# hrnr/map-merge

Measured on AMD Instinct MI355X. Metric: map-pairs/sec (normals+FPFH+SAC-IA+ICP, end to end incl. per-map features), higher is better.
Workload: dtype f32; 1 GPU; 16 maps x 500000 raw pts, FPFH + SAC_IA + ICP refine, 120 pairs; parallelism=one mm3d_estimate_maps_transforms call, 16 streams inside the library, points_after_filter_mean=406681, keypoints_mean=15692

## Files before the change

include/mm3d.h:

```cpp
#ifndef MM3D_H_
#define MM3D_H_

#include <stddef.h>
#include <stdint.h>

#ifdef __cplusplus
extern "C" {
#endif

typedef enum {
  MM3D_OK = 0,
  MM3D_EINVAL = -1,
  MM3D_EDEVICE = -2,
  MM3D_ENOMEM = -3,
  MM3D_EUNSUPPORTED = -4,
  MM3D_ECAPACITY = -5
} mm3d_status;

typedef enum { MM3D_DESC_PFH = 0, MM3D_DESC_PFHRGB, MM3D_DESC_FPFH, MM3D_DESC_RSD, MM3D_DESC_SHOT, MM3D_DESC_SC3D } mm3d_descriptor;
typedef enum { MM3D_KP_SIFT = 0, MM3D_KP_HARRIS } mm3d_keypoint;
typedef enum { MM3D_EST_MATCHING = 0, MM3D_EST_SAC_IA } mm3d_estimation_method;
typedef enum { MM3D_ICP_POINT_TO_POINT = 0, MM3D_ICP_POINT_TO_PLANE = 1 } mm3d_icp_method;

const char *mm3d_descriptor_name(int d);
// ... 26 lines not shown
void mm3d_params_default(mm3d_params *p);
int mm3d_params_from_command_line(int argc, const char *const *argv, mm3d_params *p);
size_t mm3d_params_to_string(const mm3d_params *p, char *buf, size_t cap);

typedef struct { int32_t index_query, index_match; float distance; } mm3d_corr;

typedef struct mm3d_ctx mm3d_ctx;
typedef struct mm3d_cloud mm3d_cloud;
typedef struct mm3d_normals mm3d_normals;
typedef struct mm3d_desc mm3d_desc;

int mm3d_create(int device, mm3d_ctx **out);
int mm3d_create_devices(const int *devices, int n_devices, mm3d_ctx **out);
int mm3d_device_count(const mm3d_ctx *ctx);
int mm3d_device_at(const mm3d_ctx *ctx, int i);
int mm3d_devices_use_rccl(const mm3d_ctx *ctx);
void mm3d_destroy(mm3d_ctx *ctx);
const char *mm3d_last_error(const mm3d_ctx *ctx);
int mm3d_last_icp_iterations(const mm3d_ctx *ctx);
int mm3d_last_icp_converged(const mm3d_ctx *ctx);
void mm3d_set_debug(mm3d_ctx *ctx, int on);
long long mm3d_debug_knn_fallback_rows(mm3d_ctx *ctx);
long long mm3d_debug_knn_rows(mm3d_ctx *ctx);
void mm3d_debug_waits(mm3d_ctx *ctx, long long out[2]);
int mm3d_debug_float_chain(mm3d_ctx *ctx, const float *incr, const unsigned *hits, int n, float *out);
int mm3d_debug_libm(mm3d_ctx *ctx, int fn, const float *x, const float *y, int n, float *out);
int mm3d_debug_pair_bins(mm3d_ctx *ctx, const float *p1, const float *n1, const float *p2, const float *n2, int n, int *out);
int mm3d_debug_sacia_queries_per_thread(int k);
int mm3d_debug_wave_primitives(mm3d_ctx *ctx, int op, const void *in, int n, void *out_new, void *out_old);
int mm3d_debug_sift_cert_octave(mm3d_ctx *ctx, const mm3d_cloud *points, double min_scale, int octave, float *val, float *bound,
                                size_t capacity, size_t *n_out);
void mm3d_debug_sift_cert_stats(long long out[8], int reset);
void mm3d_debug_sift_cert_min(int n);
float mm3d_debug_cloud_voxel_leaf(const mm3d_cloud *cloud);
void mm3d_debug_sacia_stats(long long out[4], int reset, int collect);
int mm3d_debug_desc_knn(mm3d_ctx *ctx, const float *a, size_t na, const float *b, size_t nb, int dim, int k, int *idx, float *d2);
typedef struct mm3d_nn_search_info {
  float max_d2;
  float rmax;
  float cell;
  float origin[3];
  int dims[3];
  int max_ring;
  int n_items;
} mm3d_nn_search_info;
int mm3d_debug_nn_search(mm3d_ctx *ctx, const mm3d_cloud *source, const mm3d_cloud *target, const float T[16], double range,
                         int convention, int split, int *idx, float *d2, mm3d_nn_search_info *info);
void mm3d_srand(mm3d_ctx *ctx, unsigned seed);
int mm3d_set_streams(mm3d_ctx *ctx, int n_streams);
int mm3d_get_streams(const mm3d_ctx *ctx);
int mm3d_last_run_stage_seconds(const mm3d_ctx *ctx, double *features_s, double *total_s);
int mm3d_last_run_device_seconds(const mm3d_ctx *ctx, double *exchange_s, double *pairs_s, double *gather_s);
size_t mm3d_last_run_map_sizes(const mm3d_ctx *ctx, size_t *points, size_t *keypoints, size_t capacity);
int mm3d_set_map_cache(mm3d_ctx *ctx, int max_maps);
int mm3d_get_map_cache(const mm3d_ctx *ctx);
void mm3d_map_cache_clear(mm3d_ctx *ctx);
int mm3d_map_cache_stats(const mm3d_ctx *ctx, long long out[6], int reset);
int mm3d_set_icp_method(mm3d_ctx *ctx, int method);
int mm3d_get_icp_method(const mm3d_ctx *ctx);
typedef enum { MM3D_ALIGN_SAC_IA = 0, MM3D_ALIGN_PREREJECTIVE = 1 } mm3d_align_method;
typedef struct mm3d_alignment_options {
  int method;
  int samples;
  int k;
  double similarity;
  double inlier_fraction;
// ... 374 lines not shown
```

map-merge_amd/__init__.py:

```python
from __future__ import annotations

import ctypes as C
import enum
import os
import subprocess

import numpy as np

_HERE = os.path.dirname(os.path.abspath(__file__))
LIB_PATH = os.environ.get("MM3D_LIB") or os.path.join(_HERE, "libmm3d.so")

POINT = np.dtype([("x", "<f4"), ("y", "<f4"), ("z", "<f4"), ("rgba", "<u4")])
NORMAL = np.dtype([("nx", "<f4"), ("ny", "<f4"), ("nz", "<f4"), ("curvature", "<f4")])
CORR = np.dtype([("index_query", "<i4"), ("index_match", "<i4"), ("distance", "<f4")])
PAIR = np.dtype([("source_idx", "<u8"), ("target_idx", "<u8"), ("transform", "<f4", (16,)),
                 ("confidence", "<f8"), ("icp_iterations", "<i4"), ("n_correspondences", "<i4"),
                 ("n_inliers", "<i4"), ("icp_correspondences", "<i4")])


class Mm3dError(RuntimeError):
    def __init__(self, status, msg):
        super().__init__(f"mm3d status {status}: {msg}")
        self.status = status

# ... 729 lines not shown

    def knnMeanDistances(self, points: "Cloud", mean_k: int) -> np.ndarray:
        out = np.empty(len(points), dtype=np.float64)
        self._ck(lib().mm3d_knn_mean_distances(self._h, points._h, int(mean_k), out.ctypes.data_as(C.c_void_p), C.c_size_t(len(out))))
        return out

    def removeOutliersStatistical(self, cloud: "Cloud", mean_k: int = 16, stddev_mult: float = 2.0) -> "Cloud":
        h = C.c_void_p()
        self._ck(lib().mm3d_remove_outliers_statistical(self._h, cloud._h, int(mean_k), C.c_double(stddev_mult), C.byref(h)))
        return Cloud(self, h)

    def clusterLabels(self, points: "Cloud", tolerance: float, with_stats: bool = False):
        out = np.empty(len(points), dtype=np.int32)
        st = ClusterStats()
        self._ck(lib().mm3d_cluster_labels(self._h, points._h, C.c_double(tolerance), out.ctypes.data_as(C.c_void_p), C.c_size_t(len(out)),
                                           C.byref(st)))
        return (out, st.as_dict()) if with_stats else out

    def removeSmallClusters(self, cloud: "Cloud", tolerance: float, method=ClusterMethod.MIN_SIZE, min_size: int = 100) -> "Cloud":
        h = C.c_void_p()
        self._ck(lib().mm3d_remove_small_clusters(self._h, cloud._h, C.c_double(tolerance), int(method), int(min_size), C.byref(h)))
        return Cloud(self, h)

    def siftCertOctave(self, points: "Cloud", min_scale: float, octave: int):
        n = C.c_size_t(0)
        self._ck(lib().mm3d_debug_sift_cert_octave(self._h, points._h, C.c_double(min_scale), int(octave), None, None, C.c_size_t(0), C.byref(n)))
        if n.value == 0:
            return None
        val = np.empty((n.value, 5), dtype=np.float32)
        bound = np.empty((n.value, 5), dtype=np.float32)
        self._ck(lib().mm3d_debug_sift_cert_octave(self._h, points._h, C.c_double(min_scale), int(octave), val.ctypes.data_as(C.c_void_p),
                                                   bound.ctypes.data_as(C.c_void_p), C.c_size_t(n.value), C.byref(n)))
        return val, bound

    def harrisResponse(self, points: "Cloud", normals: "Normals", radius: float) -> np.ndarray:
        out = np.zeros(max(len(points), 1), dtype=np.float32)
        self._ck(lib().mm3d_harris_response(self._h, points._h, normals._h, C.c_double(radius), out.ctypes.data_as(C.c_void_p)))
        return out[:len(points)]

    def computeLocalDescriptors(self, points: "Cloud", normals: "Normals", keypoints: "Cloud", descriptor,
                                feature_radius: float) -> "Descriptors":
        h = C.c_void_p()
        self._ck(lib().mm3d_compute_descriptors(self._h, points._h, normals._h, keypoints._h, int(descriptor),
                                                C.c_double(feature_radius), C.byref(h)))
        return Descriptors(self, h)

    def findFeatureCorrespondences(self, source: "Descriptors", target: "Descriptors", k: int = 5):
        n = C.c_size_t()
        self._ck(lib().mm3d_find_correspondences(self._h, source._h, target._h, C.c_size_t(k), None, C.c_size_t(0),
                                                 C.byref(n)))
        out = np.empty(max(n.value, 1), dtype=CORR)
        self._ck(lib().mm3d_find_correspondences(self._h, source._h, target._h, C.c_size_t(k),
                                                 out.ctypes.data_as(C.c_void_p), C.c_size_t(len(out)), C.byref(n)))
        return out[:n.value].copy()

    def estimateTransformFromCorrespondences(self, source_keypoints, target_keypoints, correspondences,
                                             inlier_threshold: float):
        corr = np.ascontiguousarray(correspondences, dtype=CORR)
        T = np.zeros(16, dtype=np.float32)
        inl = np.empty(max(len(corr), 1), dtype=CORR)
        n = C.c_size_t()
        self._ck(lib().mm3d_estimate_transform_from_correspondences(
            self._h, source_keypoints._h, target_keypoints._h, corr.ctypes.data_as(C.c_void_p), C.c_size_t(len(corr)),
            C.c_double(inlier_threshold), T.ctypes.data_as(C.c_void_p), inl.ctypes.data_as(C.c_void_p),
            C.c_size_t(len(inl)), C.byref(n)))
        return _Tout(T), inl[:n.value].copy()
# ... 539 lines not shown
```

map-merge_amd/csrc/sift.hip:

```cpp
#include <atomic>
#include <cfloat>
#include <functional>
#include <type_traits>
#include <memory>

#include "sorted_nb.hpp"
#include "snb_lds.hpp"
#include "sift_cert.hpp"

namespace mm3d {

constexpr int kScales = 6;
constexpr int kDog = 5;
constexpr int kKnn = 25;

struct SiftScales {
  float sigma_sqr[kScales];
  float thr9[kScales];
  float rcp[kScales];
};

__device__ __forceinline__ float intensity_of(float w)
{
  const unsigned c = __float_as_uint(w);
  const int r = (int)((c >> 16) & 255u), g = (int)((c >> 8) & 255u), b = (int)(c & 255u);
  return lm::fdiv_const((float)(299 * r + 587 * g + 114 * b), 1000.0f, 0.001f);
}

__global__ void __launch_bounds__(256)
k_sift_dog(const float4 *__restrict__ q_pts, const int2 *__restrict__ items, int n_items, GridView g ,
           const float4 *__restrict__ pts , float radius, float r2, SiftScales sc, SnScratch scr,
           float *__restrict__ dog )
{
  __shared__ SnLds lds[4];
  __shared__ float resp[4][kSnG][kScales];
  __shared__ uint64_t s_tab[32];
  const int lane = threadIdx.x & 63, wave = threadIdx.x >> 6;
  if (threadIdx.x < 32) lm::exp2f_tab_copy(s_tab, threadIdx.x);
  __syncthreads();
  SnLds &L = lds[wave];
  const size_t slot = (size_t)blockIdx.x * 4 + wave;
// ... 406 lines not shown
  const float r2p = nextafterf(r2, 0.0f);
  for (int i = 0; i < kScales; ++i) {
    fs.T[i] = fminf(sc.thr9[i], r2p);
    fs.c[i] = (float)(-0.5 * 1.4426950408889634074 / (double)sc.sigma_sqr[i]);
  }
  fs.TA = 0.5f * fs.T[0];
  fs.TB = 0.25f * fs.T[0];
  return fs;
}

template <class Cfg>
struct SfLaunch {
  DevBuf<int> ctl, ov_items;
  unsigned blocks = 0;
  SfLaunch(Context *c, int n_items)
  {
    const unsigned cap = (unsigned)snb_cu_count(c->device) * (unsigned)MM3D_SF_BLOCKS;
    blocks = (unsigned)std::max(1, std::min<int>(n_items, (int)cap));
    ctl = DevBuf<int>(c, sizeof(SnbCtl) / sizeof(int));
    ov_items = DevBuf<int>(c, (size_t)std::max(n_items, 1));
    MM3D_HIP(hipMemsetAsync(ctl.get(), 0, sizeof(SnbCtl), c->stream));
  }
  SnbCtl *ctl_dev() const { return reinterpret_cast<SnbCtl *>(ctl.get()); }
};

static void sift_dog_fast_launch(Context *c, const mm3d_cloud *cur, const Grid &gr, int n_items, float max_radius, const SfScales &fs,
                                 SfLaunch<SfCfgDefault> &fl, float *dogv, float *dogb, float *rlo2, float *rup2, unsigned char *need_exact)
{
  MM3D_LAUNCH(c, "sift_dog_fast", gr.n * 36.0, (k_sift_dog_fast<SfCfgDefault>), dim3(fl.blocks), dim3(64 * SfCfgDefault::kWaves), 0,
              (const float4 *)cur->hil_pts.get(), (const int2 *)cur->wave_items.get(), n_items, gr.view(), (const float4 *)cur->pts.get(), max_radius, fs,
              fl.ctl_dev(), fl.ov_items.get(), dogv, dogb, rlo2, rup2, need_exact);
}

static bool sift_octave_certified(Context *c, const mm3d_cloud *cur, const Grid &gr, int n_items, float max_radius, float r2,
                                  const SiftScales &sc, float min_contrast, int *flags, int *pos, int *h_keypoints )
{
  const int n = (int)cur->n;
  const SfScales fs = cert_scales(sc, r2);
  DevBuf<float> dogv(c, (size_t)n * kDog), dogb(c, (size_t)n * kDog), dog(c, (size_t)n * kDog);
  DevBuf<float4> dogx(c, (size_t)n * 3);
  DevBuf<unsigned char> cls(c, (size_t)n);
  const size_t z_head = sizeof(CertCounters) + 8 * sizeof(int);
  DevBuf<unsigned char> zeroed(c, z_head + 2 * (size_t)n);
  MM3D_HIP(hipMemsetAsync(zeroed.get(), 0, z_head + 2 * (size_t)n, c->stream));
  CertCounters *ctr = reinterpret_cast<CertCounters *>(zeroed.get());
  int *n_marked_dev = reinterpret_cast<int *>(zeroed.get() + sizeof(CertCounters));
  unsigned char *need_exact = zeroed.get() + z_head, *open_p = need_exact + n;
  SfLaunch<SfCfgDefault> fl(c, n_items);
  DevBuf<float> rlo2(c, (size_t)n);
  DevBuf<float> rup2(c, (size_t)n);
  sift_dog_fast_launch(c, cur, gr, n_items, max_radius, fs, fl, dogv.get(), dogb.get(), rlo2.get(), rup2.get(), need_exact);
  MM3D_LAUNCH(c, "sift_pack", n * 100.0, k_sift_pack_iv, dim3(div_up(n, 256)), dim3(256), 0, (const float *)dogv.get(), (const float *)dogb.get(), n,
              min_contrast, dogx.get(), cls.get());
  static const bool use_reject = [] { const char *e = getenv("MM3D_SIFT_NO_REJECT"); return !(e && atoi(e)); }();
  DevBuf<int> rctl(c, sizeof(SnbCtl) / sizeof(int));
  if (use_reject) {
    MM3D_HIP(hipMemsetAsync(rctl.get(), 0, sizeof(SnbCtl), c->stream));
    const unsigned rblocks = (unsigned)std::max(1, std::min<int>(n_items, snb_cu_count(c->device) * 5));
    MM3D_LAUNCH(c, "sift_reject", 0.0, k_sift_reject, dim3(rblocks), dim3(64 * SrCfg::kWaves), 0, (const float4 *)cur->hil_pts.get(),
                (const int2 *)cur->wave_items.get(), n_items, gr.view(), (const float *)rlo2.get(), (const float *)dogv.get(), (const float *)dogb.get(),
                (const float4 *)dogx.get(), n, cls.get(), reinterpret_cast<SnbCtl *>(rctl.get()), ctr);
  }
  DevBuf<int> cids(c, (size_t)n), oids2(c, (size_t)n);
  int *n_cids = n_marked_dev + 2, *n_oids = n_marked_dev + 4;
  const unsigned one_blocks = (unsigned)snb_cu_count(c->device) * 4u;
  MM3D_LAUNCH(c, "sift_collect", n * 5.0, k_sift_collect_ids, dim3(div_up(n, 256)), dim3(256), 0, (const unsigned char *)cls.get(), 7u, n, cids.get(), n_cids);
  MM3D_LAUNCH(c, "sift_extrema_one", 0.0, k_sift_extrema_one<false>, dim3(one_blocks), dim3(256), 0, (const int *)cids.get(), (const int *)n_cids,
              (const float4 *)cur->pts.get(), gr.view(), (const float *)rup2.get(), fs.T[kScales - 1], (const float4 *)dogx.get(), n, (const float *)dogv.get(),
              (const float *)dogb.get(), (const unsigned char *)cls.get(), flags, need_exact, open_p, ctr);
  DevBuf<float4> mq(c, (size_t)n);
  DevBuf<int2> mitems(c, (size_t)n);
  DevBuf<int> mids(c, (size_t)n), mident(c, (size_t)n);
  MM3D_LAUNCH(c, "sift_collect", n * 1.0, k_sift_collect, dim3(div_up(n, 256)), dim3(256), 0, (const unsigned char *)need_exact,
              (const float4 *)cur->pts.get(), n, mq.get(), mitems.get(), mids.get(), mident.get(), n_marked_dev);
  const size_t extra_lds = sizeof(float) * 64 * kScales + 256;
  SnbLaunch<SiftCfgLarge> sl(c, n, extra_lds);
  const unsigned exact_blocks = std::min(sl.blocks, 256u);
  MM3D_LAUNCH(c, "sift_dog_exact", 0.0, (k_sift_dog_lds<SiftCfgLarge, false>), dim3(exact_blocks), dim3(64 * SiftCfgLarge::kWaves), 0,
              (const float4 *)mq.get(), (const int2 *)mitems.get(), 0, gr.view(), (const float4 *)cur->pts.get(), max_radius, r2, sc, sl.ctl_dev(),
              sl.ov_items.get(), dog.get(), (int *)nullptr, (unsigned char *)nullptr, (const int *)mident.get(), (const int *)n_marked_dev, 0.0f,
              (float4 *)nullptr);
  MM3D_LAUNCH(c, "sift_pack", 0.0, k_sift_pack_marked, dim3(std::min(div_up(n, 256), 64u)), dim3(256), 0, (const int *)mids.get(), (const int *)n_marked_dev,
              (const float *)dog.get(), dogv.get(), dogb.get(), n, min_contrast, dogx.get(), cls.get(), ctr);
  MM3D_LAUNCH(c, "sift_collect", n * 1.0, k_sift_collect_ids, dim3(div_up(n, 256)), dim3(256), 0, (const unsigned char *)open_p, 1u, n, oids2.get(), n_oids);
  MM3D_LAUNCH(c, "sift_extrema_fin", 0.0, k_sift_extrema_one<true>, dim3(64), dim3(256), 0, (const int *)oids2.get(), (const int *)n_oids,
              (const float4 *)cur->pts.get(), gr.view(), (const float *)rup2.get(), fs.T[kScales - 1], (const float4 *)dogx.get(), n, (const float *)dogv.get(),
              (const float *)dogb.get(), (const unsigned char *)cls.get(), flags, need_exact, open_p, ctr);
  int *h = (int *)c->pin(64);
  MM3D_HIP(hipMemcpyAsync(h, ctr, sizeof(CertCounters), hipMemcpyDeviceToHost, c->stream));
  MM3D_HIP(hipMemcpyAsync(h + 8, n_marked_dev, sizeof(int), hipMemcpyDeviceToHost, c->stream));
  MM3D_HIP(hipMemcpyAsync(h + 9, &sl.ctl_dev()->ov_count, sizeof(int), hipMemcpyDeviceToHost, c->stream));
  MM3D_HIP(hipMemcpyAsync(h + 10, &fl.ctl_dev()->ov_count, sizeof(int), hipMemcpyDeviceToHost, c->stream));
  exclusive_scan_int(c, flags, pos, (size_t)n * 3 + 1);
  MM3D_HIP(hipMemcpyAsync(h_keypoints, pos + (size_t)n * 3, sizeof(int), hipMemcpyDeviceToHost, c->stream));
  c->sync();
  const CertCounters *hc = reinterpret_cast<const CertCounters *>(h);
  g_cert_stats[0] += 1; g_cert_stats[1] += n; g_cert_stats[2] += h[8]; g_cert_stats[3] += hc->n_open;
  g_cert_stats[5] += hc->violations; g_cert_stats[6] += hc->still_open; g_cert_stats[7] += h[10];
  static const bool snb_debug = getenv("MM3D_SNB_DEBUG") != nullptr;
  if (snb_debug)
    fprintf(stderr, "sift certified octave: n=%d items=%d rejected=%d to-search=%d marked=%d open=%d still_open=%d violations=%d exact overflow=%d fast overflow items=%d\n", n, n_items,
            hc->pad[0], hc->pad[1], h[8], hc->n_open, hc->still_open, hc->violations, h[9], h[10]);
  const bool ok = hc->still_open == 0 && hc->violations == 0 && h[9] == 0;
  if (!ok) g_cert_stats[4] += 1;
  return ok;
}


size_t debug_sift_cert_octave(Context *c, const mm3d_cloud *points, double min_scale, int octave, float *val_host, float *bound_host, size_t capacity)
{
  std::unique_ptr<mm3d_cloud> cur;
  const mm3d_cloud *input = points;
  float scale = (float)min_scale;
  for (int oct = 0; oct <= octave; ++oct) {
    std::unique_ptr<mm3d_cloud> next(downsample(c, input, (double)scale));
    cur = std::move(next);
    input = cur.get();
    if (cur->n < 25) return 0;
    if (oct < octave) scale *= 2;
  }
  const mm3d_cloud *oc = cur.get();
  float scales[kScales];
  for (int i = 0; i < kScales; ++i) scales[i] = scale * powf(2.0f, (1.0f * (float)i - 1.0f) / 3.0f);
  SiftScales sc;
  for (int i = 0; i < kScales; ++i) {
    sc.sigma_sqr[i] = powf(scales[i], 2.0f);
    sc.thr9[i] = 9 * sc.sigma_sqr[i];
    sc.rcp[i] = (float)(1.0 / (double)sc.sigma_sqr[i]);
  }
  const float max_radius = 3.0f * scales[kScales - 1];
  const float r2 = (float)((double)max_radius * (double)max_radius);
  const size_t n = oc->n;
  if (n > capacity) return n;
  cloud_hilbert(c, oc, 2.5f * scale);
  const Grid &gr = cloud_grid(c, oc, max_radius * 0.5f);
  DevBuf<float> dogv(c, n * kDog), dogb(c, n * kDog);
  DevBuf<unsigned char> mark(c, n);
  MM3D_HIP(hipMemsetAsync(mark.get(), 0, n, c->stream));
  SfLaunch<SfCfgDefault> fl(c, oc->n_wave_items);
  const SfScales fs = cert_scales(sc, r2);
  DevBuf<float> rlo2(c, n), rup2(c, n);
  sift_dog_fast_launch(c, oc, gr, oc->n_wave_items, max_radius, fs, fl, dogv.get(), dogb.get(), rlo2.get(), rup2.get(), mark.get());
  MM3D_HIP(hipMemcpyAsync(val_host, dogv.get(), n * kDog * sizeof(float), hipMemcpyDeviceToHost, c->stream));
  MM3D_HIP(hipMemcpyAsync(bound_host, dogb.get(), n * kDog * sizeof(float), hipMemcpyDeviceToHost, c->stream));
  c->sync();
  return n;
}

mm3d_cloud *detect_keypoints_sift(Context *c, const mm3d_cloud *points, double min_scale, int nr_octaves,
                                  int nr_scales, double min_contrast, double normals_radius, mm3d_normals **normals_out, float grid_cell_hint)
{
  std::unique_ptr<mm3d_normals> nrm_res;
  static const bool fuse_normals = [] { const char *e = getenv("MM3D_SIFT_NO_FUSED_NORMALS"); return !(e && atoi(e)); }();
  MM3D_REQUIRE(nr_scales == 3, "SIFT: only nr_scales_per_octave == 3 (the reference's setting) is built");
  std::vector<DevBuf<float4>> parts;
  std::vector<size_t> part_n;
  std::unique_ptr<mm3d_cloud> cur;
  const mm3d_cloud *input = points;
  float scale = (float)min_scale;
  static const bool try_identity = [] { const char *e = getenv("MM3D_SIFT_NO_IDENTITY"); return !(e && atoi(e)); }();
  for (int oct = 0; oct < nr_octaves; ++oct) {
    const mm3d_cloud *octave_cloud = nullptr;
    if (oct == 0 && try_identity && downsample_is_identity(c, input, (double)scale)) {
      octave_cloud = input;
    } else {
      std::unique_ptr<mm3d_cloud> next(downsample(c, input, (double)scale));
      cur = std::move(next);
      octave_cloud = cur.get();
    }
    input = octave_cloud;
    if (octave_cloud->n < 25) break;
    float scales[kScales];
    for (int i = 0; i < kScales; ++i)
      scales[i] = scale * powf(2.0f, (1.0f * (float)i - 1.0f) / (float)nr_scales);
    SiftScales sc;
    for (int i = 0; i < kScales; ++i) {
      sc.sigma_sqr[i] = powf(scales[i], 2.0f);
      sc.thr9[i] = 9 * sc.sigma_sqr[i];
      sc.rcp[i] = (float)(1.0 / (double)sc.sigma_sqr[i]);
// ... 95 lines not shown
                  flags.get(), pos.get(), (size_t)n * 3, kp.get());
    c->settle();
    parts.emplace_back(std::move(kp));
    part_n.push_back(nk);
    scale *= 2;
  }
  size_t total = 0;
  for (size_t v : part_n) total += v;
  DevBuf<float4> all(c, total);
  size_t off = 0;
  for (size_t i = 0; i < parts.size(); ++i) {
    if (part_n[i])
      MM3D_HIP(hipMemcpyAsync(all.get() + off, parts[i].get(), part_n[i] * 16, hipMemcpyDeviceToDevice, c->stream));
    off += part_n[i];
  }
  c->settle();
  if (normals_out) {
    if (!nrm_res) nrm_res.reset(compute_normals(c, points, normals_radius));
    *normals_out = nrm_res.release();
  }
  return cloud_from_device(c, std::move(all), total);
}

#ifdef MM3D_SNB_STATS
extern "C" void mm3d_debug_snb_stats_sift(unsigned long long *out, int reset)
{
  (void)hipDeviceSynchronize();
  (void)hipMemcpyFromSymbol(out, HIP_SYMBOL(g_snb_stats), sizeof(unsigned long long) * 32);
  if (reset) { unsigned long long z[32] = {0}; (void)hipMemcpyToSymbol(HIP_SYMBOL(g_snb_stats), z, sizeof(z)); }
}
#endif

}
```

map-merge_amd/csrc/sift_cert.hpp:

```cpp
#pragma once

#include "snb_lds.hpp"

namespace mm3d {

constexpr int kCertScales = 6, kCertDog = 5, kCertKnn = 25;

struct SfScales {
  float T[kCertScales];
  float c[kCertScales];
  float TA, TB;
};

template <int WAVES_, int TILE_CAP_>
struct SfCfg {
  static constexpr int kWaves = WAVES_;
  static constexpr int kTileCap = TILE_CAP_;
  static constexpr int kVals = 3 * kCertScales + 2;
  static_assert(WAVES_ == 8, "the reduction deals its eight sums to eight waves");
  static_assert(TILE_CAP_ * 16 >= WAVES_ * (3 * kCertScales + 2) * 64 * 4, "the partial sums reuse the tile's memory");
};
#ifndef MM3D_SF_TILE
#define MM3D_SF_TILE 2816
#endif
// ... 181 lines not shown
      if (S.ntot[kCertScales][lane] <= kCertKnn) r = sc.TA;
#pragma unroll
      for (int s = 0; s < 3; ++s)
        if (S.ntot[s][lane] <= kCertKnn) r = sc.T[s];
      rlo2[self] = r;
      float ru = INFINITY;
#pragma unroll
      for (int s = kCertScales - 1; s >= 0; --s)
        if (S.ntot[s][lane] >= kCertKnn) ru = sc.T[s];
      if (S.ntot[kCertScales][lane] >= kCertKnn) ru = sc.TA;
      if (S.ntot[kCertScales + 1][lane] >= kCertKnn) ru = sc.TB;
      rup2[self] = ru;
    }
    __syncthreads();
  }
}

__device__ __forceinline__ float cert_pred(float x)
{
  const unsigned u = __float_as_uint(x);
  if ((u & 0x7fffffffu) > 0x7f800000u || u == 0xff800000u) return x;
  if ((u & 0x7fffffffu) == 0u) return __uint_as_float(0x80000001u);
  return __uint_as_float((u & 0x80000000u) ? u + 1u : u - 1u);
}
__device__ __forceinline__ float cert_succ(float x) { return -cert_pred(-x); }

__device__ __forceinline__ void cert_interval(float v, float b, float &lo, float &hi)
{
  if (b == 0.0f) { lo = v; hi = v; return; }
  lo = cert_pred(v - b);
  hi = cert_succ(v + b);
}

__device__ __forceinline__ void cert_pack_point(const float *__restrict__ dogv, const float *__restrict__ dogb, int i, int n, float min_contrast,
                                                float4 *__restrict__ dogx, unsigned char *__restrict__ cls)
{
  float lo[kCertDog], hi[kCertDog];
#pragma unroll
  for (int s = 0; s < kCertDog; ++s) cert_interval(dogv[(size_t)i * kCertDog + s], dogb ? dogb[(size_t)i * kCertDog + s] : 0.0f, lo[s], hi[s]);
  float mnhi[3], mnlo[3], mxlo[3], mxhi[3];
  unsigned c = 0;
#pragma unroll
  for (int s = 1; s <= 3; ++s) {
    mnhi[s - 1] = fminf(hi[s], cert_pred(fminf(hi[s - 1], hi[s + 1])));
    mnlo[s - 1] = fminf(lo[s], cert_pred(fminf(lo[s - 1], lo[s + 1])));
    mxlo[s - 1] = fmaxf(lo[s], cert_succ(fmaxf(lo[s - 1], lo[s + 1])));
    mxhi[s - 1] = fmaxf(hi[s], cert_succ(fmaxf(hi[s - 1], hi[s + 1])));
    if (hi[s] >= min_contrast || lo[s] <= -min_contrast) c |= 1u << (s - 1);
    if (lo[s] >= min_contrast || hi[s] <= -min_contrast) c |= 8u << (s - 1);
  }
  dogx[i] = make_float4(mnhi[0], mnhi[1], mnhi[2], mxlo[0]);
  dogx[(size_t)n + i] = make_float4(mxlo[1], mxlo[2], mnlo[0], mnlo[1]);
  dogx[2 * (size_t)n + i] = make_float4(mnlo[2], mxhi[0], mxhi[1], mxhi[2]);
  cls[i] = (unsigned char)c;
}

struct CertCounters {
  int n_marked;
  int n_open;
  int still_open;
  int violations;
  int pad[4];
};

struct SrCfg {
  static constexpr int kWaves = 4;
  static constexpr int kTileCap = 640;
};
struct alignas(16) SrLds {
  float4 ta[SrCfg::kTileCap + 4];
  float4 tb[SrCfg::kTileCap + 4];
  float2 tc[SrCfg::kTileCap + 4];
  int off[SrCfg::kWaves][64], beg[SrCfg::kWaves][64];
  float4 qpts[64];
  unsigned rej[64];
  int n_tile[2];
  int item;
};

__global__ void __launch_bounds__(64 * SrCfg::kWaves)
k_sift_reject(const float4 *__restrict__ q_pts, const int2 *__restrict__ items, int n_items, GridView g ,
              const float *__restrict__ rlo2, const float *__restrict__ dogv, const float *__restrict__ dogb, const float4 *__restrict__ dogx, int n_pts,
              unsigned char *__restrict__ cls, SnbCtl *ctl, CertCounters *__restrict__ ctr)
{
  __shared__ SrLds S;
  constexpr int W = SrCfg::kWaves, T = 64 * W;
  const int lane = threadIdx.x & 63, wave = threadIdx.x >> 6;
// ... 94 lines not shown
        }
        unsigned bits = 0;
#pragma unroll
        for (int s = 0; s < 3; ++s) bits |= (mn[s] ? 1u << s : 0u) | (mx[s] ? 8u << s : 0u);
        if (bits && ask) atomicOr(&S.rej[lane], bits);
      }
      __syncthreads();
      if (wave == 0 && live && (c0 & 7u)) {
        const unsigned b = S.rej[lane];
        unsigned c = c0;
        int gone = 0, kept = 0;
#pragma unroll
        for (int s = 0; s < 3; ++s) {
          if (!(c0 & (1u << s))) continue;
          if ((b & (1u << s)) && (b & (8u << s))) { c &= ~((1u << s) | (8u << s)); ++gone; }
          else ++kept;
        }
        if (c != c0) cls[self] = (unsigned char)c;
        if (gone) atomicAdd(&ctr->pad[0], gone);
        if (kept) atomicAdd(&ctr->pad[1], kept);
      }
    }
    __syncthreads();
  }
}

__global__ void k_sift_pack_iv(const float *__restrict__ dogv, const float *__restrict__ dogb, int n, float min_contrast,
                               float4 *__restrict__ dogx, unsigned char *__restrict__ cls)
{
  const int i = blockIdx.x * blockDim.x + threadIdx.x;
  if (i < n) cert_pack_point(dogv, dogb, i, n, min_contrast, dogx, cls);
}


__global__ void k_sift_pack_marked(const int *__restrict__ ids, const int *__restrict__ n_ids, const float *__restrict__ dog,
                                   float *__restrict__ dogv, float *__restrict__ dogb, int n, float min_contrast,
                                   float4 *__restrict__ dogx, unsigned char *__restrict__ cls, CertCounters *__restrict__ ctr)
{
  const int total = *n_ids;
  for (int k = blockIdx.x * blockDim.x + threadIdx.x; k < total; k += gridDim.x * blockDim.x) {
    const int i = ids[k];
    bool bad = false;
#pragma unroll
    for (int s = 0; s < kCertDog; ++s) {
      const float ex = dog[(size_t)i * kCertDog + s];
      float lo, hi;
      cert_interval(dogv[(size_t)i * kCertDog + s], dogb[(size_t)i * kCertDog + s], lo, hi);
      if (!(ex >= lo && ex <= hi)) bad = true;
      dogv[(size_t)i * kCertDog + s] = ex;
      dogb[(size_t)i * kCertDog + s] = 0.0f;
    }
    if (bad) atomicAdd(&ctr->violations, 1);
    cert_pack_point(dogv, dogb, i, n, min_contrast, dogx, cls);
  }
}

__global__ void k_sift_collect(const unsigned char *__restrict__ mark, const float4 *__restrict__ pts, int n, float4 *__restrict__ q,
                               int2 *__restrict__ items, int *__restrict__ ids, int *__restrict__ ident, int *__restrict__ count)
{
  const int i = blockIdx.x * blockDim.x + threadIdx.x;
  if (i >= n || !mark[i]) return;
  const int k = atomicAdd(count, 1);
  const float4 p = pts[i];
  q[k] = make_float4(p.x, p.y, p.z, __int_as_float(i));
  items[k] = make_int2(k, 1);
  ids[k] = i;
  ident[k] = k;
}

__global__ void k_sift_collect_ids(const unsigned char *__restrict__ sel, unsigned mask, int n, int *__restrict__ ids, int *__restrict__ n_ids)
{
  const int i = blockIdx.x * blockDim.x + threadIdx.x;
  if (i < n && (sel[i] & mask)) ids[atomicAdd(n_ids, 1)] = i;
}

template <bool kFinal>
__global__ void __launch_bounds__(256)
k_sift_extrema_one(const int *__restrict__ ids, const int *__restrict__ n_ids_dev, const float4 *__restrict__ pts , GridView g ,
                   const float *__restrict__ rup2, float r2_max , const float4 *__restrict__ dogx , int n_pts,
                   const float *__restrict__ dogv,
                   const float *__restrict__ dogb, const unsigned char *__restrict__ cls, int *__restrict__ flags ,
                   unsigned char *__restrict__ need_exact, unsigned char *__restrict__ open_p, CertCounters *__restrict__ ctr)
{
  __shared__ int s_off[4][65];
  __shared__ int s_beg[4][64];
  const int lane = threadIdx.x & 63, wave = threadIdx.x >> 6;
  const int n_ids = *n_ids_dev;
  const int n_waves = (int)gridDim.x * 4;
  int *w_off = s_off[wave], *w_beg = s_beg[wave];
  for (int k = (int)blockIdx.x * 4 + wave; k < n_ids; k += n_waves) {
    const int self = ids[k];
    const float4 q = pts[self];
    float r2q = rup2 ? rup2[self] : INFINITY;
    const unsigned c = cls[self];
    const unsigned cand = c & 7u, live = (c >> 3) & 7u;
    if (!cand) continue;
    if (!(r2q < INFINITY)) {
      const int kk0 = g.n < kCertKnn ? g.n : kCertKnn;
      float r2 = r2_max;
      for (int grow = 0; grow < 48; ++grow) {
        r2 *= 4.0f;
// ... 156 lines not shown
```

Baseline: 1404 map-pairs/s.

## Replace exact SIFT DoG path with one block-per-point sorted-neighbour kernel

The exact difference-of-Gaussians recompute for uncertified points used to gather queries, run the general sorted-neighbour LDS kernel, and then apply a separate pack kernel. It is now one kernel that handles one marked point per block. The kernel collects in-radius neighbours in distance order, using radix-histogram windows and a bitonic sort in LDS so the summation order stays deterministic. It then does the certificate check and packing inline. This removes several launches, intermediate buffers and the full-size dog array, but adds repeated neighbour scans when a point has more than 2048 neighbours and an overflow failure path that skips the point.

```diff
diff --git a/include/mm3d.h b/include/mm3d.h
--- a/include/mm3d.h
+++ b/include/mm3d.h
@@ -82,6 +82,8 @@
                                 size_t capacity, size_t *n_out);
 void mm3d_debug_sift_cert_stats(long long out[8], int reset);
 void mm3d_debug_sift_cert_min(int n);
+int mm3d_debug_sift_dog_marked(mm3d_ctx *ctx, const mm3d_cloud *points, double min_scale, int octave, const int *ids, size_t n_ids,
+                               int small_capacity, float *out);
 float mm3d_debug_cloud_voxel_leaf(const mm3d_cloud *cloud);
 void mm3d_debug_sacia_stats(long long out[4], int reset, int collect);
 int mm3d_debug_desc_knn(mm3d_ctx *ctx, const float *a, size_t na, const float *b, size_t nb, int dim, int k, int *idx, float *d2);
diff --git a/map-merge_amd/__init__.py b/map-merge_amd/__init__.py
--- a/map-merge_amd/__init__.py
+++ b/map-merge_amd/__init__.py
@@ -785,6 +785,13 @@
         self._ck(lib().mm3d_debug_sift_cert_octave(self._h, points._h, C.c_double(min_scale), int(octave), val.ctypes.data_as(C.c_void_p),
                                                    bound.ctypes.data_as(C.c_void_p), C.c_size_t(n.value), C.byref(n)))
         return val, bound
+
+    def siftDogMarked(self, points: "Cloud", min_scale: float, octave: int, ids, small_capacity: bool = False) -> np.ndarray:
+        ids = np.ascontiguousarray(ids, dtype=np.int32)
+        out = np.full((len(ids), 5), np.nan, dtype=np.float32)
+        self._ck(lib().mm3d_debug_sift_dog_marked(self._h, points._h, C.c_double(min_scale), int(octave), ids.ctypes.data_as(C.c_void_p),
+                                                  C.c_size_t(len(ids)), 1 if small_capacity else 0, out.ctypes.data_as(C.c_void_p)))
+        return out
 
     def harrisResponse(self, points: "Cloud", normals: "Normals", radius: float) -> np.ndarray:
         out = np.zeros(max(len(points), 1), dtype=np.float32)
diff --git a/map-merge_amd/csrc/sift.hip b/map-merge_amd/csrc/sift.hip
--- a/map-merge_amd/csrc/sift.hip
+++ b/map-merge_amd/csrc/sift.hip
@@ -1,5 +1,6 @@
 #include <atomic>
 #include <cfloat>
+#include <climits>
 #include <functional>
 #include <type_traits>
 #include <memory>
@@ -7,6 +8,7 @@
 #include "sorted_nb.hpp"
 #include "snb_lds.hpp"
 #include "sift_cert.hpp"
+#include "capi_guard.hpp"
 
 namespace mm3d {
 
@@ -479,12 +481,210 @@
               fl.ctl_dev(), fl.ov_items.get(), dogv, dogb, rlo2, rup2, need_exact);
 }
 
+template <int K>
+struct alignas(16) SmLds {
+  unsigned long long key[K];
+  float term[2 * kScales][257];
+  uint64_t tab[32];
+  unsigned hist[256];
+  float sum[2 * kScales];
+  int cnt;
+  unsigned edge;
+};
+constexpr int kMarkedCap = 2048, kMarkedCapSmall = 128;
+static_assert(sizeof(SmLds<kMarkedCap>) <= 32768, "k_sift_dog_marked shares a CU with the other streams' kernels");
+
+template <int K>
+__global__ void __launch_bounds__(256)
+k_sift_dog_marked(const int *__restrict__ ids, const int *__restrict__ n_ids_dev, const float4 *__restrict__ pts ,
+                  GridView g , float radius, float r2, SiftScales sc,
+                  float *__restrict__ raw_out ,
+                  float *__restrict__ dogv, float *__restrict__ dogb, int n, float min_contrast, float4 *__restrict__ dogx,
+                  unsigned char *__restrict__ cls, CertCounters *__restrict__ ctr, int *__restrict__ overflow )
+{
+  static_assert(K >= 2 && (K & (K - 1)) == 0, "the sort works on a power of two");
+  __shared__ SmLds<K> S;
+  const int tid = threadIdx.x, lane = tid & 63, wave = tid >> 6;
+  if (tid < 32) lm::exp2f_tab_copy(S.tab, tid);
+  const int n_ids = *n_ids_dev;
+  const unsigned r2b = __float_as_uint(r2);
+  const float ri = radius * 1.0001f + 1e-4f;
+  for (int k = (int)blockIdx.x; k < n_ids; k += (int)gridDim.x) {
+    const int self = ids[k];
+    const float4 q = pts[self];
+    const int x0 = max(cell_floor(q.x - ri, g.minx, g.inv), 0), x1 = min(cell_floor(q.x + ri, g.minx, g.inv), g.dx - 1);
+    const int y0 = max(cell_floor(q.y - ri, g.miny, g.inv), 0), y1 = min(cell_floor(q.y + ri, g.miny, g.inv), g.dy - 1);
+    const int z0 = max(cell_floor(q.z - ri, g.minz, g.inv), 0), z1 = min(cell_floor(q.z + ri, g.minz, g.inv), g.dz - 1);
+    const int ny = y1 - y0 + 1, nz = z1 - z0 + 1;
+    const int nrows = (x0 <= x1 && ny > 0 && nz > 0) ? ny * nz : 0;
+    auto visit = [&](auto &&f) {
+      for (int r = wave; r < nrows; r += 4) {
+        const int z = z0 + r / ny, y = y0 + r % ny;
+        const int row = (z * g.dy + y) * g.dx;
+        const int b = g.cell_start[row + x0], e = g.cell_start[row + x1 + 1];
+        for (int j0 = b; j0 < e; j0 += kWave) {
+          const int j = j0 + lane;
+          const bool in = j < e;
+          const float4 cd = g.pts[in ? j : b];
+          const float d2 = dist2(q.x, q.y, q.z, cd.x, cd.y, cd.z);
+          f(in && d2 < r2, __float_as_uint(d2), __float_as_uint(cd.w));
+        }
+      }
+    };
+    auto block_total = [&](int mine) {
+      __syncthreads();
+      if (tid == 0) S.cnt = 0;
+      __syncthreads();
+      const int w = wave_sum(mine);
+      if (lane == 0 && w) atomicAdd(&S.cnt, w);
+      __syncthreads();
+      return S.cnt;
+    };
+    float acc = 0.0f;
+    unsigned lo = 0u;
+    bool failed = false;
+    for (;;) {
+      int mine = 0;
+      visit([&](bool mem, unsigned bits, unsigned) { mine += (mem && bits >= lo) ? 1 : 0; });
+      const int rem = block_total(mine);
+      unsigned hi = r2b;
+      if (rem > K) {
+        unsigned hp = 0u;
+        int base = 0;
+        for (int sh = 24; sh >= 0; sh -= 8) {
+          __syncthreads();
+          S.hist[tid] = 0u;
+          __syncthreads();
+          visit([&](bool mem, unsigned bits, unsigned) {
+            if (mem && bits >= lo && (sh == 24 || (bits >> (sh + 8)) == (hp >> (sh + 8)))) atomicAdd(&S.hist[(bits >> sh) & 255u], 1u);
+          });
+          __syncthreads();
+          if (tid == 0) {
+            int a = base;
+            unsigned d = 0u;
+            for (unsigned j = 0; j < 255u; ++j) {
+              const int nxt = a + (int)S.hist[j];
+              if (nxt > K) break;
+              a = nxt;
+              d = j + 1u;
+            }
+            S.edge = d;
+            S.cnt = a;
+          }
+          __syncthreads();
+          hp |= S.edge << sh;
+          base = S.cnt;
+        }
+        hi = hp;
+        if (hi <= lo) { failed = true; break; }
+      }
+      __syncthreads();
+      if (tid == 0) S.cnt = 0;
+      __syncthreads();
+      visit([&](bool mem, unsigned bits, unsigned idx) {
+        const bool kp = mem && bits >= lo && bits < hi;
+        const unsigned long long m = ballot(kp);
+        if (m) {
+          int b0 = 0;
+          if (lane == 0) b0 = atomicAdd(&S.cnt, __popcll(m));
+          b0 = __builtin_amdgcn_readfirstlane(b0);
+          const int d = snb_mbcnt(m, b0);
+          if (kp && d < K) S.key[d] = ((unsigned long long)bits << 32) | idx;
+        }
+      });
+      __syncthreads();
+      const int m = S.cnt;
+      if (m > K) { failed = true; break; }
+      if (m > 0) {
+        int P = 2;
+        while (P < m) P <<= 1;
+        for (int i = m + tid; i < P; i += 256) S.key[i] = ~0ull;
+        __syncthreads();
+        for (int kk = 2; kk <= P; kk <<= 1) {
+          for (int j = kk >> 1; j > 0; j >>= 1) {
+            for (int i = tid; i < P; i += 256) {
+              const int ixj = i ^ j;
+              if (ixj > i) {
+                const unsigned long long a = S.key[i], b = S.key[ixj];
+                if ((a > b) == ((i & kk) == 0)) { S.key[i] = b; S.key[ixj] = a; }
+              }
+            }
+            __syncthreads();
+          }
+        }
+        for (int c0 = 0; c0 < m; c0 += 256) {
+          const int e = c0 + tid;
+          float tv[kScales], tw[kScales];
+#pragma unroll
+          for (int s = 0; s < kScales; ++s) { tv[s] = 0.0f; tw[s] = 0.0f; }
+          if (e < m) {
+            const unsigned long long key = S.key[e];
+            const float d2 = __uint_as_float((unsigned)(key >> 32));
+            const float val = intensity_of(pts[(unsigned)key].w);
+#pragma unroll
+            for (int s = 0; s < kScales; ++s) {
+              if (d2 <= sc.thr9[s]) {
+                const float w = lm::expf_glibc_t<false>(lm::fdiv_const(-0.5f * d2, sc.sigma_sqr[s], sc.rcp[s]), [&](unsigned i) { return S.tab[i]; });
+                tw[s] = w;
+                tv[s] = __fmul_rn(val, w);
+              }
+            }
+          }
+#pragma unroll
+          for (int s = 0; s < kScales; ++s) { S.term[s][tid] = tv[s]; S.term[kScales + s][tid] = tw[s]; }
+          __syncthreads();
+          if (tid < 2 * kScales) {
+            const int cn = min(256, m - c0);
+            const float *t = S.term[tid];
+            for (int u = 0; u < cn; ++u) acc = __fadd_rn(acc, t[u]);
+          }
+          __syncthreads();
+        }
+      }
+      if (hi == r2b) break;
+      lo = hi;
+    }
+    if (failed) {
+      if (tid == 0) atomicAdd(overflow, 1);
+      continue;
+    }
+    if (tid < 2 * kScales) S.sum[tid] = acc;
+    __syncthreads();
+    if (tid == 0) {
+      float ex[kDog];
+      float prev = S.sum[0] / S.sum[kScales];
+#pragma unroll
+      for (int s = 1; s < kScales; ++s) {
+        const float cur = S.sum[s] / S.sum[kScales + s];
+        ex[s - 1] = cur - prev;
+        prev = cur;
+      }
+      if (raw_out) {
+#pragma unroll
+        for (int s = 0; s < kDog; ++s) raw_out[(size_t)k * kDog + s] = ex[s];
+      } else {
+        bool bad = false;
+#pragma unroll
+        for (int s = 0; s < kDog; ++s) {
+          float l, h;
+          cert_interval(dogv[(size_t)self * kDog + s], dogb[(size_t)self * kDog + s], l, h);
+          if (!(ex[s] >= l && ex[s] <= h)) bad = true;
+          dogv[(size_t)self * kDog + s] = ex[s];
+          dogb[(size_t)self * kDog + s] = 0.0f;
+        }
+        if (bad) atomicAdd(&ctr->violations, 1);
+        cert_pack_bounds(ex, ex, self, n, min_contrast, dogx, cls);
+      }
+    }
+  }
+}
+
 static bool sift_octave_certified(Context *c, const mm3d_cloud *cur, const Grid &gr, int n_items, float max_radius, float r2,
                                   const SiftScales &sc, float min_contrast, int *flags, int *pos, int *h_keypoints )
 {
   const int n = (int)cur->n;
   const SfScales fs = cert_scales(sc, r2);
-  DevBuf<float> dogv(c, (size_t)n * kDog), dogb(c, (size_t)n * kDog), dog(c, (size_t)n * kDog);
+  DevBuf<float> dogv(c, (size_t)n * kDog), dogb(c, (size_t)n * kDog);
   DevBuf<float4> dogx(c, (size_t)n * 3);
   DevBuf<unsigned char> cls(c, (size_t)n);
   const size_t z_head = sizeof(CertCounters) + 8 * sizeof(int);
@@ -515,20 +715,13 @@
   MM3D_LAUNCH(c, "sift_extrema_one", 0.0, k_sift_extrema_one<false>, dim3(one_blocks), dim3(256), 0, (const int *)cids.get(), (const int *)n_cids,
               (const float4 *)cur->pts.get(), gr.view(), (const float *)rup2.get(), fs.T[kScales - 1], (const float4 *)dogx.get(), n, (const float *)dogv.get(),
               (const float *)dogb.get(), (const unsigned char *)cls.get(), flags, need_exact, open_p, ctr);
-  DevBuf<float4> mq(c, (size_t)n);
-  DevBuf<int2> mitems(c, (size_t)n);
-  DevBuf<int> mids(c, (size_t)n), mident(c, (size_t)n);
-  MM3D_LAUNCH(c, "sift_collect", n * 1.0, k_sift_collect, dim3(div_up(n, 256)), dim3(256), 0, (const unsigned char *)need_exact,
-              (const float4 *)cur->pts.get(), n, mq.get(), mitems.get(), mids.get(), mident.get(), n_marked_dev);
-  const size_t extra_lds = sizeof(float) * 64 * kScales + 256;
-  SnbLaunch<SiftCfgLarge> sl(c, n, extra_lds);
-  const unsigned exact_blocks = std::min(sl.blocks, 256u);
-  MM3D_LAUNCH(c, "sift_dog_exact", 0.0, (k_sift_dog_lds<SiftCfgLarge, false>), dim3(exact_blocks), dim3(64 * SiftCfgLarge::kWaves), 0,
-              (const float4 *)mq.get(), (const int2 *)mitems.get(), 0, gr.view(), (const float4 *)cur->pts.get(), max_radius, r2, sc, sl.ctl_dev(),
-              sl.ov_items.get(), dog.get(), (int *)nullptr, (unsigned char *)nullptr, (const int *)mident.get(), (const int *)n_marked_dev, 0.0f,
-              (float4 *)nullptr);
-  MM3D_LAUNCH(c, "sift_pack", 0.0, k_sift_pack_marked, dim3(std::min(div_up(n, 256), 64u)), dim3(256), 0, (const int *)mids.get(), (const int *)n_marked_dev,
-              (const float *)dog.get(), dogv.get(), dogb.get(), n, min_contrast, dogx.get(), cls.get(), ctr);
+  DevBuf<int> mids(c, (size_t)n);
+  int *n_ov_marked = n_marked_dev + 6;
+  MM3D_LAUNCH(c, "sift_collect", n * 1.0, k_sift_collect_ids, dim3(div_up(n, 256)), dim3(256), 0, (const unsigned char *)need_exact, 0xffu, n, mids.get(),
+              n_marked_dev);
+  MM3D_LAUNCH(c, "sift_dog_marked", 0.0, (k_sift_dog_marked<kMarkedCap>), dim3(256), dim3(256), 0, (const int *)mids.get(), (const int *)n_marked_dev,
+              (const float4 *)cur->pts.get(), gr.view(), max_radius, r2, sc, (float *)nullptr, dogv.get(), dogb.get(), n, min_contrast, dogx.get(),
+              cls.get(), ctr, n_ov_marked);
   MM3D_LAUNCH(c, "sift_collect", n * 1.0, k_sift_collect_ids, dim3(div_up(n, 256)), dim3(256), 0, (const unsigned char *)open_p, 1u, n, oids2.get(), n_oids);
   MM3D_LAUNCH(c, "sift_extrema_fin", 0.0, k_sift_extrema_one<true>, dim3(64), dim3(256), 0, (const int *)oids2.get(), (const int *)n_oids,
               (const float4 *)cur->pts.get(), gr.view(), (const float *)rup2.get(), fs.T[kScales - 1], (const float4 *)dogx.get(), n, (const float *)dogv.get(),
@@ -536,7 +729,7 @@
   int *h = (int *)c->pin(64);
   MM3D_HIP(hipMemcpyAsync(h, ctr, sizeof(CertCounters), hipMemcpyDeviceToHost, c->stream));
   MM3D_HIP(hipMemcpyAsync(h + 8, n_marked_dev, sizeof(int), hipMemcpyDeviceToHost, c->stream));
-  MM3D_HIP(hipMemcpyAsync(h + 9, &sl.ctl_dev()->ov_count, sizeof(int), hipMemcpyDeviceToHost, c->stream));
+  MM3D_HIP(hipMemcpyAsync(h + 9, n_ov_marked, sizeof(int), hipMemcpyDeviceToHost, c->stream));
   MM3D_HIP(hipMemcpyAsync(h + 10, &fl.ctl_dev()->ov_count, sizeof(int), hipMemcpyDeviceToHost, c->stream));
   exclusive_scan_int(c, flags, pos, (size_t)n * 3 + 1);
   MM3D_HIP(hipMemcpyAsync(h_keypoints, pos + (size_t)n * 3, sizeof(int), hipMemcpyDeviceToHost, c->stream));
@@ -554,29 +747,42 @@
 }
 
 
-size_t debug_sift_cert_octave(Context *c, const mm3d_cloud *points, double min_scale, int octave, float *val_host, float *bound_host, size_t capacity)
-{
-  std::unique_ptr<mm3d_cloud> cur;
+struct DebugOctave {
+  std::unique_ptr<mm3d_cloud> cloud;
+  SiftScales sc;
+  float scale, max_radius, r2;
+};
+static bool debug_octave(Context *c, const mm3d_cloud *points, double min_scale, int octave, DebugOctave &o)
+{
   const mm3d_cloud *input = points;
   float scale = (float)min_scale;
   for (int oct = 0; oct <= octave; ++oct) {
     std::unique_ptr<mm3d_cloud> next(downsample(c, input, (double)scale));
-    cur = std::move(next);
-    input = cur.get();
-    if (cur->n < 25) return 0;
+    o.cloud = std::move(next);
+    input = o.cloud.get();
+    if (o.cloud->n < 25) return false;
     if (oct < octave) scale *= 2;
   }
-  const mm3d_cloud *oc = cur.get();
   float scales[kScales];
   for (int i = 0; i < kScales; ++i) scales[i] = scale * powf(2.0f, (1.0f * (float)i - 1.0f) / 3.0f);
-  SiftScales sc;
   for (int i = 0; i < kScales; ++i) {
-    sc.sigma_sqr[i] = powf(scales[i], 2.0f);
-    sc.thr9[i] = 9 * sc.sigma_sqr[i];
-    sc.rcp[i] = (float)(1.0 / (double)sc.sigma_sqr[i]);
-  }
-  const float max_radius = 3.0f * scales[kScales - 1];
-  const float r2 = (float)((double)max_radius * (double)max_radius);
+    o.sc.sigma_sqr[i] = powf(scales[i], 2.0f);
+    o.sc.thr9[i] = 9 * o.sc.sigma_sqr[i];
+    o.sc.rcp[i] = (float)(1.0 / (double)o.sc.sigma_sqr[i]);
+  }
+  o.scale = scale;
+  o.max_radius = 3.0f * scales[kScales - 1];
+  o.r2 = (float)((double)o.max_radius * (double)o.max_radius);
+  return true;
+}
+
+size_t debug_sift_cert_octave(Context *c, const mm3d_cloud *points, double min_scale, int octave, float *val_host, float *bound_host, size_t capacity)
+{
+  DebugOctave o;
+  if (!debug_octave(c, points, min_scale, octave, o)) return 0;
+  const mm3d_cloud *oc = o.cloud.get();
+  const SiftScales &sc = o.sc;
+  const float scale = o.scale, max_radius = o.max_radius, r2 = o.r2;
   const size_t n = oc->n;
   if (n > capacity) return n;
   cloud_hilbert(c, oc, 2.5f * scale);
@@ -592,6 +798,40 @@
   MM3D_HIP(hipMemcpyAsync(bound_host, dogb.get(), n * kDog * sizeof(float), hipMemcpyDeviceToHost, c->stream));
   c->sync();
   return n;
+}
+
+static void debug_sift_dog_marked(Context *c, const mm3d_cloud *points, double min_scale, int octave, const int *ids, size_t n_ids, int small_capacity,
+                                  float *out)
+{
+  if (n_ids == 0) return;
+  DebugOctave o;
+  if (!debug_octave(c, points, min_scale, octave, o)) throw Error(MM3D_EINVAL, "mm3d_debug_sift_dog_marked: no such octave");
+  const mm3d_cloud *oc = o.cloud.get();
+  MM3D_REQUIRE(oc->n_finite == oc->n, "mm3d_debug_sift_dog_marked: the octave cloud holds non-finite points");
+  for (size_t i = 0; i < n_ids; ++i)
+    if (ids[i] < 0 || (size_t)ids[i] >= oc->n) throw Error(MM3D_EINVAL, "mm3d_debug_sift_dog_marked: an id outside the octave cloud");
+  MM3D_REQUIRE(n_ids <= (size_t)INT_MAX / kDog, "mm3d_debug_sift_dog_marked: too many ids");
+  const Grid &gr = cloud_grid(c, oc, o.max_radius * 0.5f);
+  DevBuf<int> d_ids(c, n_ids), d_ctl(c, 2);
+  DevBuf<float> d_out(c, n_ids * kDog);
+  int *h_ctl = (int *)c->pin(64), *h_ov = h_ctl + 2;
+  h_ctl[0] = (int)n_ids;
+  h_ctl[1] = 0;
+  MM3D_HIP(hipMemcpyAsync(d_ids.get(), ids, n_ids * sizeof(int), hipMemcpyHostToDevice, c->stream));
+  MM3D_HIP(hipMemcpyAsync(d_ctl.get(), h_ctl, 2 * sizeof(int), hipMemcpyHostToDevice, c->stream));
+  MM3D_HIP(hipMemcpyAsync(d_out.get(), out, n_ids * kDog * sizeof(float), hipMemcpyHostToDevice, c->stream));
+  if (small_capacity)
+    MM3D_LAUNCH(c, "sift_dog_marked", 0.0, (k_sift_dog_marked<kMarkedCapSmall>), dim3(256), dim3(256), 0, (const int *)d_ids.get(), (const int *)d_ctl.get(),
+                (const float4 *)oc->pts.get(), gr.view(), o.max_radius, o.r2, o.sc, d_out.get(), (float *)nullptr, (float *)nullptr, (int)oc->n, 0.0f,
+                (float4 *)nullptr, (unsigned char *)nullptr, (CertCounters *)nullptr, d_ctl.get() + 1);
+  else
+    MM3D_LAUNCH(c, "sift_dog_marked", 0.0, (k_sift_dog_marked<kMarkedCap>), dim3(256), dim3(256), 0, (const int *)d_ids.get(), (const int *)d_ctl.get(),
+                (const float4 *)oc->pts.get(), gr.view(), o.max_radius, o.r2, o.sc, d_out.get(), (float *)nullptr, (float *)nullptr, (int)oc->n, 0.0f,
+                (float4 *)nullptr, (unsigned char *)nullptr, (CertCounters *)nullptr, d_ctl.get() + 1);
+  MM3D_HIP(hipMemcpyAsync(out, d_out.get(), n_ids * kDog * sizeof(float), hipMemcpyDeviceToHost, c->stream));
+  MM3D_HIP(hipMemcpyAsync(h_ov, d_ctl.get() + 1, sizeof(int), hipMemcpyDeviceToHost, c->stream));
+  c->sync();
+  if (*h_ov > 0) throw Error(MM3D_EUNSUPPORTED, "mm3d_debug_sift_dog_marked: a point has more neighbours at one distance than the sort buffer holds");
 }
 
 mm3d_cloud *detect_keypoints_sift(Context *c, const mm3d_cloud *points, double min_scale, int nr_octaves,
@@ -753,3 +993,11 @@
 #endif
 
 }
+
+extern "C" int mm3d_debug_sift_dog_marked(mm3d_ctx *ctx, const mm3d_cloud *points, double min_scale, int octave, const int *ids, size_t n_ids,
+                                          int small_capacity, float *out)
+{
+  if (!points || !(min_scale > 0.0) || !std::isfinite(min_scale) || octave < 0 || octave > 16) return MM3D_EINVAL;
+  if (n_ids && (!ids || !out)) return MM3D_EINVAL;
+  return mm3d::guarded(ctx, [&] { mm3d::debug_sift_dog_marked(ctx, points, min_scale, octave, ids, n_ids, small_capacity, out); });
+}
diff --git a/map-merge_amd/csrc/sift_cert.hpp b/map-merge_amd/csrc/sift_cert.hpp
--- a/map-merge_amd/csrc/sift_cert.hpp
+++ b/map-merge_amd/csrc/sift_cert.hpp
@@ -237,12 +237,9 @@
   hi = cert_succ(v + b);
 }
 
-__device__ __forceinline__ void cert_pack_point(const float *__restrict__ dogv, const float *__restrict__ dogb, int i, int n, float min_contrast,
-                                                float4 *__restrict__ dogx, unsigned char *__restrict__ cls)
-{
-  float lo[kCertDog], hi[kCertDog];
-#pragma unroll
-  for (int s = 0; s < kCertDog; ++s) cert_interval(dogv[(size_t)i * kCertDog + s], dogb ? dogb[(size_t)i * kCertDog + s] : 0.0f, lo[s], hi[s]);
+__device__ __forceinline__ void cert_pack_bounds(const float (&lo)[kCertDog], const float (&hi)[kCertDog], int i, int n, float min_contrast,
+                                                 float4 *__restrict__ dogx, unsigned char *__restrict__ cls)
+{
   float mnhi[3], mnlo[3], mxlo[3], mxhi[3];
   unsigned c = 0;
 #pragma unroll
@@ -258,6 +255,15 @@
   dogx[(size_t)n + i] = make_float4(mxlo[1], mxlo[2], mnlo[0], mnlo[1]);
   dogx[2 * (size_t)n + i] = make_float4(mnlo[2], mxhi[0], mxhi[1], mxhi[2]);
   cls[i] = (unsigned char)c;
+}
+
+__device__ __forceinline__ void cert_pack_point(const float *__restrict__ dogv, const float *__restrict__ dogb, int i, int n, float min_contrast,
+                                                float4 *__restrict__ dogx, unsigned char *__restrict__ cls)
+{
+  float lo[kCertDog], hi[kCertDog];
+#pragma unroll
+  for (int s = 0; s < kCertDog; ++s) cert_interval(dogv[(size_t)i * kCertDog + s], dogb ? dogb[(size_t)i * kCertDog + s] : 0.0f, lo[s], hi[s]);
+  cert_pack_bounds(lo, hi, i, n, min_contrast, dogx, cls);
 }
 
 struct CertCounters {
@@ -418,41 +424,6 @@
   if (i < n) cert_pack_point(dogv, dogb, i, n, min_contrast, dogx, cls);
 }
 
-
-__global__ void k_sift_pack_marked(const int *__restrict__ ids, const int *__restrict__ n_ids, const float *__restrict__ dog,
-                                   float *__restrict__ dogv, float *__restrict__ dogb, int n, float min_contrast,
-                                   float4 *__restrict__ dogx, unsigned char *__restrict__ cls, CertCounters *__restrict__ ctr)
-{
-  const int total = *n_ids;
-  for (int k = blockIdx.x * blockDim.x + threadIdx.x; k < total; k += gridDim.x * blockDim.x) {
-    const int i = ids[k];
-    bool bad = false;
-#pragma unroll
-    for (int s = 0; s < kCertDog; ++s) {
-      const float ex = dog[(size_t)i * kCertDog + s];
-      float lo, hi;
-      cert_interval(dogv[(size_t)i * kCertDog + s], dogb[(size_t)i * kCertDog + s], lo, hi);
-      if (!(ex >= lo && ex <= hi)) bad = true;
-      dogv[(size_t)i * kCertDog + s] = ex;
-      dogb[(size_t)i * kCertDog + s] = 0.0f;
-    }
-    if (bad) atomicAdd(&ctr->violations, 1);
-    cert_pack_point(dogv, dogb, i, n, min_contrast, dogx, cls);
-  }
-}
-
-__global__ void k_sift_collect(const unsigned char *__restrict__ mark, const float4 *__restrict__ pts, int n, float4 *__restrict__ q,
-                               int2 *__restrict__ items, int *__restrict__ ids, int *__restrict__ ident, int *__restrict__ count)
-{
-  const int i = blockIdx.x * blockDim.x + threadIdx.x;
-  if (i >= n || !mark[i]) return;
-  const int k = atomicAdd(count, 1);
-  const float4 p = pts[i];
-  q[k] = make_float4(p.x, p.y, p.z, __int_as_float(i));
-  items[k] = make_int2(k, 1);
-  ids[k] = i;
-  ident[k] = k;
-}
 
 __global__ void k_sift_collect_ids(const unsigned char *__restrict__ sel, unsigned mask, int n, int *__restrict__ ids, int *__restrict__ n_ids)
 {
```

Measured after the change: 1425 map-pairs/s (median of 6 runs). +1.5%, better.
